# Yawning/secp256k1-voi

Hardware: AMD Instinct MI355X
Metric: secp256k1 ECDSA verifications/sec at batch=2^20 per GPU (higher is better)
Workload: dtype u32; 1 GPU; 2^20 ECDSA verifies (u1*G+u2*P per lane) per GPU (BASELINE config 2), 65536 distinct keys per GPU, all valid, low-s; parallelism=shard1, inputs=resident in HBM, collective=one all-gather per step: bitmap shard + valid count of every rank, gt_bits=26, gt_bits_at_first_call=20, gt_bytes=43822088192, numa_node=1, cpus_bound=128

## Files before the change

### include/secp256k1_voi_amd.h

```cpp
#ifndef SECP256K1_VOI_AMD_H
#define SECP256K1_VOI_AMD_H

#include <stddef.h>
#include <stdint.h>

#ifdef __cplusplus
extern "C" {
#endif

typedef struct s2k_ctx s2k_ctx;

enum {
  S2K_OK = 0,
  S2K_ERR_NO_DEVICE = -1,
  S2K_ERR_HIP = -2,
  S2K_ERR_ARG = -3,
  S2K_ERR_NOMEM = -4,
  S2K_PENDING = 1
};

#define S2K_ECDSA_REJECT_MALLEABLE 1u
#define S2K_ECDSA_FORCE_COMPLETE 0x80000000u
#define S2K_ECDSA_FORCE_WORKLIST 0x40000000u

// ... 330 lines not shown
int s2k_ct_scalar_set_bytes(const uint8_t src32[32], uint8_t out32[32], uint64_t *did_reduce);
int s2k_ct_fe_op(int op, const uint8_t a32[32], const uint8_t b32[32], uint8_t out32[32], uint64_t *flag);
uint64_t s2k_ct_debug_fe_mul_count(void);

enum {
  S2K_OP_MUL = 0,
  S2K_OP_SQR = 1,
  S2K_OP_ADD = 2,
  S2K_OP_SUB = 3,
  S2K_OP_NEG = 4,
  S2K_OP_INV = 5,
  S2K_OP_SQRT = 6
};
int s2k_fp_op_batch(s2k_ctx *ctx, int op, size_t n, const uint8_t *a, const uint8_t *b, uint8_t *out, uint8_t *flag);
int s2k_fn_op_batch(s2k_ctx *ctx, int op, size_t n, const uint8_t *a, const uint8_t *b, uint8_t *out, uint8_t *flag);
int s2k_fn_split_glv_batch(s2k_ctx *ctx, size_t n, const uint8_t *k, uint8_t *k1, uint8_t *k2);

enum {
  S2K_HP_MUL = 0, S2K_HP_SQR, S2K_HP_MUL_PLUS, S2K_HP_SQR_PLUS, S2K_HP_MUL_ADD_MUL, S2K_HP_MUL_ADD_SQR,
  S2K_HP_ADD, S2K_HP_NEGATE, S2K_HP_HALF, S2K_HP_NORMALIZE, S2K_HP_COND_NEGATE1, S2K_HP_INV, S2K_HP_SQRT,
  S2K_HP_EQ, S2K_HP_MUL_SMALL21, S2K_HP_NORMALIZE_WEAK, S2K_HP_JDBL, S2K_HP_JADD, S2K_HP_PT29_DBL,
  S2K_HP_PT29_ADD, S2K_HP_PT29_ADD_MIXED,
  S2K_HP_INV_GCD,
  S2K_HP_JADD_FULL,
  S2K_HP_PT29Q_DBL, S2K_HP_PT29Q_ADD,
  S2K_HP_XYZZ_ADD,
  S2K_HP_XYZZ_ROUND,
  S2K_HP_FER_MUL, S2K_HP_FER_MUL_PLUS, S2K_HP_FER_MUL_ADD_MUL, S2K_HP_FER_SMALL, S2K_HP_PT29R_DBL, S2K_HP_PT29R_ADD, S2K_HP_FER_SWAPS,
  S2K_HP_SC26_MUL, S2K_HP_SC26_SQR, S2K_HP_SC26_TO_MONT, S2K_HP_SC26_TO_SC, S2K_HP_SC26_INV, S2K_HP_SC26_CHAIN,
  S2K_HP_SC_MONTMUL, S2K_HP_SC_TO_MONT, S2K_HP_SC_MONT_INV, S2K_HP_SC_ADD, S2K_HP_SC_NEG, S2K_HP_SC_REDUCE_ONCE,
  S2K_HP_SC_GT_HALF_N,
  S2K_HP_AFF_DBL, S2K_HP_AFF_ADD,
  S2K_HP_XYZZ_ADD_FIRST,
  S2K_HP_PT29R_ADD_B3
};
int s2k_fp_op_batch_ex(s2k_ctx *ctx, uint32_t impl, int op, uint32_t lazy, size_t n, const uint8_t *const in[5],
                       uint8_t *out, uint8_t *out2, uint8_t *flag);
int s2k_fn_split_glv_batch_ex(s2k_ctx *ctx, uint32_t impl, size_t n, const uint8_t *k, uint8_t *k1, uint8_t *k2,
                              uint8_t *signs);

int s2k_generator_window_bits(void);
int s2k_debug_gtable_entry(s2k_ctx *ctx, unsigned i, unsigned d, uint8_t *out64);

#ifdef __cplusplus
}
#endif
#endif
```

### secp256k1_voi_amd/__init__.py

```python
from __future__ import annotations

import ctypes as C
import os
import subprocess

import numpy as np

if "GPU_MAX_HW_QUEUES" not in os.environ:
    os.environ["GPU_MAX_HW_QUEUES"] = "8"
    import sys as _sys
    _t = _sys.modules.get("torch")
    if _t is not None and getattr(_t, "cuda", None) is not None and _t.cuda.is_initialized():
        import warnings
        warnings.warn("secp256k1_voi_amd: the HIP runtime was initialised before this package was imported, so "
                      "GPU_MAX_HW_QUEUES=8 comes too late; streams of the engine may share hardware queues "
                      "(export GPU_MAX_HW_QUEUES=8 in the environment instead)", RuntimeWarning)

_HERE = os.path.dirname(os.path.abspath(__file__))
LIB_PATH = os.environ.get("S2K_LIB") or os.path.join(_HERE, "libsecp256k1_voi_amd.so")
CSRC = os.path.join(_HERE, "csrc")

REJECT_MALLEABLE = 1
BIP0066 = 2
FORCE_COMPLETE = 0x80000000
FORCE_WORKLIST = 0x40000000
ENCODING_ASN1, ENCODING_COMPACT, ENCODING_COMPACT_RECOVERABLE = 0, 1, 2

OP_MUL, OP_SQR, OP_ADD, OP_SUB, OP_NEG, OP_INV, OP_SQRT = range(7)
IMPL_COMPLETE, IMPL_FAST = 0, 1
CTX_WAIT_TABLES = 1
KEYS_OFF, KEYS_AUTO, KEYS_ALWAYS, KEYS_ADAPTIVE = 0, 1, 2, 3
LADDER_COMB, LADDER_WINDOW = 0, 1
KEYSET_AUTO, KEYSET_CHUNKS, KEYSET_JOINT, KEYSET_JOINT5, KEYSET_JOINT6, KEYSET_COMB = 0, 1, 2, 3, 4, 5
(HP_MUL, HP_SQR, HP_MUL_PLUS, HP_SQR_PLUS, HP_MUL_ADD_MUL, HP_MUL_ADD_SQR, HP_ADD, HP_NEGATE, HP_HALF, HP_NORMALIZE,
 HP_COND_NEGATE1, HP_INV, HP_SQRT, HP_EQ, HP_MUL_SMALL21, HP_NORMALIZE_WEAK, HP_JDBL, HP_JADD, HP_PT29_DBL, HP_PT29_ADD,
 HP_PT29_ADD_MIXED, HP_INV_GCD, HP_JADD_FULL, HP_PT29Q_DBL, HP_PT29Q_ADD, HP_XYZZ_ADD, HP_XYZZ_ROUND,
 HP_FER_MUL, HP_FER_MUL_PLUS, HP_FER_MUL_ADD_MUL, HP_FER_SMALL, HP_PT29R_DBL, HP_PT29R_ADD, HP_FER_SWAPS,
 HP_SC26_MUL, HP_SC26_SQR, HP_SC26_TO_MONT, HP_SC26_TO_SC, HP_SC26_INV, HP_SC26_CHAIN,
 HP_SC_MONTMUL, HP_SC_TO_MONT, HP_SC_MONT_INV, HP_SC_ADD, HP_SC_NEG, HP_SC_REDUCE_ONCE, HP_SC_GT_HALF_N,
 HP_AFF_DBL, HP_AFF_ADD, HP_XYZZ_ADD_FIRST, HP_PT29R_ADD_B3) = range(51)
KEYSET_LADDER_LANE, KEYSET_LADDER_ROW = 0, 1
H2C_SSWU_RO, H2C_SSWU_NU = 0, 1

IDENTITY = bytes(65)


def pinned_array(shape, dtype=np.uint8) -> np.ndarray:
    import weakref
    lib = load_library()
    nbytes = int(np.prod(shape)) * np.dtype(dtype).itemsize
    p = lib.s2k_host_alloc(max(nbytes, 1))
    if not p:
        raise EngineError("s2k_host_alloc failed")
    buf = (C.c_uint8 * max(nbytes, 1)).from_address(p)
    weakref.finalize(buf, lib.s2k_host_free, p)
    return np.frombuffer(buf, dtype=dtype, count=int(np.prod(shape))).reshape(shape)


def page_aligned_array(shape, dtype=np.uint8) -> np.ndarray:
    import mmap
    nbytes = int(np.prod(shape)) * np.dtype(dtype).itemsize
    page = mmap.PAGESIZE
    m = mmap.mmap(-1, max((nbytes + page - 1) // page * page, page))
    return np.frombuffer(m, dtype=dtype, count=int(np.prod(shape))).reshape(shape)


def host_register(a: np.ndarray) -> None:
    import mmap
    lib = load_library()
    nbytes, base = a.nbytes, a
    while getattr(base, "base", None) is not None:
        base = base.base
    if isinstance(base, memoryview):
# ... 191 lines not shown
    lib.s2k_group_keyset_create.argtypes = [vp, sz, vp, ci, vp]
    lib.s2k_group_keyset_destroy.argtypes = [vp]
    lib.s2k_group_keyset_destroy.restype = None
    lib.s2k_group_keyset_size.argtypes = [vp]
    lib.s2k_group_keyset_size.restype = sz
    lib.s2k_group_keyset_layout.argtypes = [vp]
    lib.s2k_group_keyset_device_bytes.argtypes = [vp]
    lib.s2k_group_keyset_device_bytes.restype = sz
    lib.s2k_group_ecdsa_verify_batch_keyset.argtypes = [vp, vp, sz, vp, vp, vp, vp, u32, vp]
    lib.s2k_group_ecdsa_verify_batch_keyset_submit.argtypes = [vp, vp, sz, vp, vp, vp, vp, u32, vp, vp]
    lib.s2k_group_ecdsa_verify_batch.argtypes = [vp, sz, vp, vp, vp, vp, u32, vp]
    lib.s2k_group_ecdsa_verify_batch_submit.argtypes = [vp, sz, vp, vp, vp, vp, u32, vp, C.POINTER(u64)]
    lib.s2k_group_wait.argtypes = [vp, u64]
    lib.s2k_group_ecdsa_verify_encoded_batch.argtypes = [vp, sz, vp, vp, vp, vp, vp, vp, ci, sz, u32, vp]
    lib.s2k_group_ecdsa_verify_encoded_batch_submit.argtypes = [vp, sz, vp, vp, vp, vp, vp, vp, ci, sz, u32, vp, C.POINTER(u64)]
    lib.s2k_group_member_stats.argtypes = [vp, vp]
    lib.s2k_schnorr_verify_batch.argtypes = [vp, sz, vp, vp, vp, sz, vp, u32, vp]
    lib.s2k_schnorr_verify_batch_device.argtypes = [vp, sz, vp, vp, vp, sz, vp, u32, vp, vp]
    lib.s2k_schnorr_verify_batch_keyset.argtypes = [vp, vp, sz, vp, vp, vp, sz, vp, u32, vp]
    lib.s2k_schnorr_verify_batch_keyset_device.argtypes = [vp, vp, sz, vp, vp, vp, sz, vp, u32, vp, vp]
    lib.s2k_schnorr_verify_batch_keyset_submit.argtypes = [vp, vp, sz, vp, vp, vp, sz, vp, u32, vp, vp]
    lib.s2k_schnorr_verify_batch_keyset_bykey.argtypes = [vp, vp, sz, vp, vp, vp, sz, vp, u32, vp]
    lib.s2k_schnorr_verify_batch_keyset_bykey_device.argtypes = [vp, vp, sz, vp, vp, vp, sz, vp, u32, vp, vp]
    lib.s2k_schnorr_verify_batch_keyset_bykey_submit.argtypes = [vp, vp, sz, vp, vp, vp, sz, vp, u32, vp, vp]
    lib.s2k_schnorr_batch_verify_rlc.argtypes = [vp, sz, vp, vp, vp, sz, vp, vp, C.POINTER(ci)]
    lib.s2k_schnorr_batch_verify_rlc_device.argtypes = [vp, sz, vp, vp, vp, sz, vp, vp, C.POINTER(ci), vp]
    lib.s2k_schnorr_verify_batch_bisect.argtypes = [vp, sz, vp, vp, vp, sz, vp, vp, vp, vp]
    lib.s2k_schnorr_verify_batch_bisect_device.argtypes = [vp, sz, vp, vp, vp, sz, vp, vp, vp, vp, vp]
    lib.s2k_scalar_base_mult_batch.argtypes = [vp, sz, vp, vp]
    lib.s2k_scalar_mult_batch.argtypes = [vp, sz, vp, vp, vp]
    lib.s2k_double_scalar_mult_basepoint_batch.argtypes = [vp, sz, vp, vp, vp, vp]
    lib.s2k_double_scalar_mult_basepoint_batch_ex.argtypes = [vp, u32, sz, vp, vp, vp, vp]
    lib.s2k_fp_op_batch_ex.argtypes = [vp, u32, ci, u32, sz, vp, vp, vp, vp]
    lib.s2k_fn_split_glv_batch_ex.argtypes = [vp, u32, sz, vp, vp, vp, vp]
    lib.s2k_point_add_batch.argtypes = [vp, sz, vp, vp, vp]
    lib.s2k_point_double_batch.argtypes = [vp, sz, vp, vp]
    lib.s2k_point_decode_batch.argtypes = [vp, sz, sz, vp, vp, vp]
    lib.s2k_multi_scalar_mult.argtypes = [vp, sz, vp, vp, vp]
    lib.s2k_multi_scalar_mult_device.argtypes = [vp, sz, vp, vp, vp, vp]
    lib.s2k_multi_scalar_mult_segments.argtypes = [vp, sz, vp, vp, sz, vp, vp]
    lib.s2k_multi_scalar_mult_segments_device.argtypes = [vp, sz, vp, vp, sz, vp, vp, vp]
    lib.s2k_debug_msm_segments_plan.argtypes = [sz, sz, vp, u32, C.c_uint64, vp, sz, vp, vp, vp, vp]
    lib.s2k_pointset_create.argtypes = [vp, sz, vp, ci, C.POINTER(vp)]
    lib.s2k_pointset_destroy.argtypes = [vp]
    lib.s2k_pointset_destroy.restype = None
    lib.s2k_pointset_size.argtypes = [vp]
    lib.s2k_pointset_size.restype = sz
    lib.s2k_pointset_window_bits.argtypes = [vp]
    lib.s2k_pointset_device_bytes.argtypes = [vp]
    lib.s2k_pointset_device_bytes.restype = sz
    lib.s2k_pointset_geometry.argtypes = [ci, vp]
    lib.s2k_keyset_geometry.argtypes = [ci, vp]
    lib.s2k_debug_pointset_entry.argtypes = [vp, sz, C.c_uint, C.c_uint, vp]
    lib.s2k_debug_pointset_check_args.argtypes = [sz, sz, ci, sz, vp]
    lib.s2k_pointset_multi_scalar_mult_segments.argtypes = [vp, vp, sz, vp, vp, sz, vp, vp]
    lib.s2k_pointset_multi_scalar_mult_segments_device.argtypes = [vp, vp, sz, vp, vp, sz, vp, vp, vp]
    lib.s2k_h2c_dst_prime.argtypes = [C.c_char_p, sz, C.c_char_p, C.POINTER(sz)]
    lib.s2k_expand_message_xmd_batch.argtypes = [vp, sz, C.c_char_p, sz, vp, vp, sz, sz, vp]
    lib.s2k_map_to_curve_batch.argtypes = [vp, sz, sz, sz, vp, vp]
    lib.s2k_hash_to_curve_batch.argtypes = [vp, ci, sz, C.c_char_p, sz, vp, vp, sz, vp]
    lib.s2k_hash_to_curve_batch_device.argtypes = [vp, ci, sz, C.c_char_p, sz, vp, vp, sz, sz, vp, vp]
    lib.s2k_fp_op_batch.argtypes = [vp, ci, sz, vp, vp, vp, vp]
    lib.s2k_fn_op_batch.argtypes = [vp, ci, sz, vp, vp, vp, vp]
    lib.s2k_fn_split_glv_batch.argtypes = [vp, sz, vp, vp, vp]
    lib.s2k_debug_gtable_entry.argtypes = [vp, C.c_uint, C.c_uint, vp]
    lib.s2k_ct_scalar_mult.argtypes = [C.c_char_p, C.c_char_p, C.c_char_p]
# ... 58 lines not shown
    "s2k_ctx_set_key_grouping", "s2k_ctx_set_keyed_ladder", "s2k_ctx_last_keyed_ladder", "s2k_ctx_key_grouping_stats", "s2k_ctx_key_grouping_adaptive",
    "s2k_ecdsa_verify_batch", "s2k_ecdsa_verify_batch_device", "s2k_ecdsa_workspace_bytes", "s2k_ctx_device_bytes",
    "s2k_keyset_create", "s2k_keyset_create_ex", "s2k_keyset_layout", "s2k_keyset_geometry", "s2k_keyset_destroy", "s2k_keyset_size", "s2k_keyset_device_bytes", "s2k_keyset_valid_keys",
    "s2k_ecdsa_verify_batch_keyset", "s2k_ecdsa_verify_batch_keyset_device", "s2k_ecdsa_verify_batch_keyset_submit",
    "s2k_keyset_index_geometry", "s2k_keyset_index_create", "s2k_keyset_index_info", "s2k_keyset_lookup", "s2k_keyset_lookup_device",
    "s2k_ecdsa_verify_batch_keyset_bykey", "s2k_ecdsa_verify_batch_keyset_bykey_device", "s2k_ecdsa_verify_batch_keyset_bykey_submit",
    "s2k_schnorr_verify_batch_keyset_bykey", "s2k_schnorr_verify_batch_keyset_bykey_device", "s2k_schnorr_verify_batch_keyset_bykey_submit",
    "s2k_pack_valid_device", "s2k_host_alloc", "s2k_host_free", "s2k_host_register", "s2k_host_unregister", "s2k_ecdsa_recover_batch", "s2k_ecdsa_recover_batch_device",
    "s2k_ecdsa_batch_verify_rlc", "s2k_ecdsa_batch_verify_rlc_device",
    "s2k_ecdsa_verify_recoverable_batch_bisect", "s2k_ecdsa_verify_recoverable_batch_bisect_device",
    "s2k_parse_asn1_signature", "s2k_parse_compact_signature", "s2k_is_valid_signature_encoding_bip0066",
    "s2k_ecdsa_verify_encoded_batch",
    "s2k_ecdsa_verify_encoded_batch_keyset", "s2k_ecdsa_verify_encoded_batch_keyset_submit", "s2k_ctx_last_encoded_keyset_stats",
    "s2k_ecdsa_verify_batch_submit", "s2k_ecdsa_verify_encoded_batch_submit", "s2k_wait", "s2k_poll", "s2k_wait_all",
    "s2k_device_count", "s2k_group_create", "s2k_group_destroy", "s2k_group_size", "s2k_group_last_error",
    "s2k_group_set_key_grouping", "s2k_group_set_small_batch_max", "s2k_group_set_mid_batch_max", "s2k_group_ecdsa_verify_batch", "s2k_group_ecdsa_verify_batch_submit", "s2k_group_wait",
    "s2k_group_ecdsa_verify_encoded_batch", "s2k_group_ecdsa_verify_encoded_batch_submit",
    "s2k_group_member_stats", "s2k_group_schnorr_batch_verify_rlc", "s2k_group_multi_scalar_mult",
    "s2k_group_keyset_create", "s2k_group_keyset_destroy", "s2k_group_keyset_size", "s2k_group_keyset_layout", "s2k_group_keyset_device_bytes",
    "s2k_group_ecdsa_verify_batch_keyset", "s2k_group_ecdsa_verify_batch_keyset_submit",
    "s2k_schnorr_verify_batch", "s2k_schnorr_verify_batch_device",
    "s2k_schnorr_verify_batch_keyset", "s2k_schnorr_verify_batch_keyset_device", "s2k_schnorr_verify_batch_keyset_submit",
    "s2k_schnorr_batch_verify_rlc", "s2k_schnorr_batch_verify_rlc_device",
    "s2k_schnorr_verify_batch_bisect", "s2k_schnorr_verify_batch_bisect_device",
    "s2k_scalar_base_mult_batch", "s2k_scalar_mult_batch", "s2k_double_scalar_mult_basepoint_batch",
    "s2k_point_add_batch", "s2k_point_double_batch", "s2k_point_decode_batch",
    "s2k_multi_scalar_mult", "s2k_multi_scalar_mult_device",
    "s2k_multi_scalar_mult_segments", "s2k_multi_scalar_mult_segments_device", "s2k_debug_msm_segments_plan",
    "s2k_pointset_create", "s2k_pointset_destroy", "s2k_pointset_size", "s2k_pointset_window_bits", "s2k_pointset_device_bytes",
    "s2k_pointset_geometry", "s2k_debug_pointset_entry", "s2k_debug_pointset_check_args",
    "s2k_pointset_multi_scalar_mult_segments", "s2k_pointset_multi_scalar_mult_segments_device",
    "s2k_h2c_dst_prime", "s2k_expand_message_xmd_batch", "s2k_map_to_curve_batch", "s2k_hash_to_curve_batch", "s2k_hash_to_curve_batch_device",
    "s2k_fp_op_batch", "s2k_fn_op_batch", "s2k_fn_split_glv_batch", "s2k_debug_gtable_entry", "s2k_generator_window_bits",
    "s2k_double_scalar_mult_basepoint_batch_ex", "s2k_fp_op_batch_ex", "s2k_fn_split_glv_batch_ex",
    "s2k_ct_scalar_mult", "s2k_ct_scalar_base_mult", "s2k_ct_ecdh", "s2k_ct_ecdsa_sign_raw", "s2k_ct_debug_fe_mul_count",
    "s2k_ct_multi_scalar_mult",
    "s2k_device_pci_bus_id", "s2k_device_numa_node", "s2k_bind_thread_to_node", "s2k_topology_prefer_node", "s2k_topology_node_count",
    "s2k_topology_numa_node_of_pci", "s2k_topology_node_cpus", "s2k_ctx_ticket_timing", "s2k_ticket_times",
    "s2k_group_member_stats_ex", "s2k_group_gt_wait", "s2k_group_shard_size", "s2k_group_host_alloc", "s2k_group_host_free",
    "s2k_ctx_set_small_batch_max", "s2k_ctx_set_mid_batch_max", "s2k_ctx_create_ex", "s2k_set_generator_table_budget", "s2k_set_table_memory_budgets", "s2k_ctx_gt_info", "s2k_ctx_gt_note", "s2k_ctx_gt_wait",
    "s2k_group_create_ex", "s2k_debug_gt_swap_in_call",
    "s2k_ctx_set_keyset_small_batch_max", "s2k_ctx_last_keyset_ladder", "s2k_group_set_keyset_small_batch_max",
    "s2k_ct_point_add", "s2k_ct_point_double", "s2k_ct_point_subtract", "s2k_ct_point_negate", "s2k_ct_point_conditional_negate",
    "s2k_ct_point_conditional_select", "s2k_ct_point_equal", "s2k_ct_point_is_identity", "s2k_ct_point_is_y_odd",
    "s2k_ct_scalar_op", "s2k_ct_scalar_conditional_select", "s2k_ct_scalar_conditional_negate", "s2k_ct_scalar_predicate",
    "s2k_ct_scalar_set_bytes", "s2k_ct_fe_op",
]


def _arr(x, width, n=None):
    if isinstance(x, (list, tuple)):
        x = b"".join(x)
    if isinstance(x, (bytes, bytearray, memoryview)):
        a = np.frombuffer(bytes(x), dtype=np.uint8)
    else:
        a = np.ascontiguousarray(x, dtype=np.uint8).reshape(-1)
    if a.size % width:
        raise ValueError(f"buffer length {a.size} is not a multiple of {width}")
    a = a.reshape(-1, width)
    if n is not None and a.shape[0] != n:
        raise ValueError(f"length mismatch: expected {n} items, got {a.shape[0]}")
    return np.ascontiguousarray(a)


def parse_asn1_signature(der: bytes):
    r, s = C.create_string_buffer(32), C.create_string_buffer(32)
    return (r.raw, s.raw) if load_library().s2k_parse_asn1_signature(der, len(der), r, s) == 0 else None
# ... 796 lines not shown
        out = self._points_out(n)
        self._check(self._lib.s2k_scalar_mult_batch(self._h, n, k.ctypes.data, points.ctypes.data, out.ctypes.data))
        return out

    def double_scalar_mult_basepoint_batch(self, u1, u2, points):
        u1 = _arr(u1, 32)
        n = u1.shape[0]
        u2, points = _arr(u2, 32, n), _arr(points, 65, n)
        out = self._points_out(n)
        self._check(self._lib.s2k_double_scalar_mult_basepoint_batch(self._h, n, u1.ctypes.data, u2.ctypes.data,
                                                                     points.ctypes.data, out.ctypes.data))
        return out

    def double_scalar_mult_basepoint_batch_ex(self, impl, u1, u2, points):
        u2 = _arr(u2, 32)
        n = u2.shape[0]
        points = _arr(points, 65, n)
        u1a = _arr(u1, 32, n) if u1 is not None else None
        out = self._points_out(n)
        self._check(self._lib.s2k_double_scalar_mult_basepoint_batch_ex(self._h, impl, n,
                                                                        u1a.ctypes.data if u1a is not None else None,
                                                                        u2.ctypes.data, points.ctypes.data, out.ctypes.data))
        return out

    def fp_op_batch_ex(self, op, operands, lazy=0):
        ops = [(_arr(x, 32) if x is not None else None) for x in operands] + [None] * (5 - len(operands))
        n = ops[0].shape[0]
        ptrs = (C.c_void_p * 5)(*[(x.ctypes.data if x is not None else None) for x in ops])
        out, out2, flag = (np.zeros((n, 32), dtype=np.uint8), np.zeros((n, 32), dtype=np.uint8), np.zeros(n, dtype=np.uint8))
        self._check(self._lib.s2k_fp_op_batch_ex(self._h, IMPL_FAST, op, lazy, n, ptrs, out.ctypes.data, out2.ctypes.data,
                                                 flag.ctypes.data))
        return out, out2, flag

    def fn_split_glv_odd_batch(self, k):
        k = _arr(k, 32)
        n = k.shape[0]
        k1, k2, sg = np.zeros((n, 32), np.uint8), np.zeros((n, 32), np.uint8), np.zeros(n, np.uint8)
        self._check(self._lib.s2k_fn_split_glv_batch_ex(self._h, IMPL_FAST, n, k.ctypes.data, k1.ctypes.data, k2.ctypes.data,
                                                        sg.ctypes.data))
        return k1, k2, sg

    def point_add_batch(self, a, b):
        a = _arr(a, 65)
        n = a.shape[0]
        b = _arr(b, 65, n)
        out = self._points_out(n)
        self._check(self._lib.s2k_point_add_batch(self._h, n, a.ctypes.data, b.ctypes.data, out.ctypes.data))
        return out

    def point_double_batch(self, a):
        a = _arr(a, 65)
        out = self._points_out(a.shape[0])
        self._check(self._lib.s2k_point_double_batch(self._h, a.shape[0], a.ctypes.data, out.ctypes.data))
        return out

    def multi_scalar_mult(self, scalars, points) -> bytes:
        scalars = _arr(scalars, 32)
        n = scalars.shape[0]
        points = _arr(points, 65, n)
        out = np.zeros(65, dtype=np.uint8)
        self._check(self._lib.s2k_multi_scalar_mult(self._h, n, scalars.ctypes.data if n else None,
                                                    points.ctypes.data if n else None, out.ctypes.data))
        return out.tobytes()

    def multi_scalar_mult_device(self, n, d_scalars, d_points, d_out65, stream=0):
        self._check(self._lib.s2k_multi_scalar_mult_device(self._h, int(n), d_scalars, d_points, d_out65, stream))
# ... 417 lines not shown
```

### secp256k1_voi_amd/csrc/engine.hip

```cpp
#include <hip/hip_runtime.h>

#include <cstdarg>
#include <cstdio>
#include <cstdlib>
#include <cstring>
#include <new>

#include <sys/random.h>
#include <unistd.h>

#include <atomic>
#include <chrono>
#include <condition_variable>
#include <mutex>
#include <thread>

#include "engine_internal.h"
#include "keyset_index.h"
#include "fe.h"
#include "fe29_inv.h"
#include "jacobian29.h"
#include "xyzz29.h"
#include "lane_tables.h"
#include "pt29.h"
// ... 619 lines not shown
    const uint4* kt = kg.ktab + (size_t)kg.ptab[idx] * (G::SLOTS * 8);
    {
      fe29 lx, ly;
      ke_load_xy(kt + (size_t)(neg1 == neg2 ? G::LEAD : G::LEAD + 1) * 8, false, lx, ly);
      acc.x = lx;
      acc.y = fe29_cond_negate1(ly, neg1);
      acc.z = fe29_one();
    }
    __shared__ uint32_t cols[G::SPACING][256];
    {
      uint32_t t1[G::TEETH], t2[G::TEETH];
#pragma unroll
      for (int t = 0; t < G::TEETH; ++t) {
        const int bit = G::SPACING * t + 1, limb = bit >> 5, sh = bit & 31;
        uint32_t v1 = k1.v[limb] >> sh, v2 = k2.v[limb] >> sh;
        if (sh > 32 - G::SPACING) {
          v1 |= k1.v[limb + 1] << (32 - sh);
          v2 |= k2.v[limb + 1] << (32 - sh);
        }
        t1[t] = v1 & ((1u << G::SPACING) - 1u);
        t2[t] = v2 & ((1u << G::SPACING) - 1u);
      }
#pragma unroll
      for (int j = 0; j < G::SPACING; ++j) {
        uint32_t w = 0;
#pragma unroll
        for (int t = 0; t < G::TEETH; ++t) w |= (((t1[t] >> j) & 1u) << t) | (((t2[t] >> j) & 1u) << (8 + t));
        cols[j][threadIdx.x] = w;
      }
    }
#pragma unroll 1
    for (int j = G::SPACING - 1;; --j) {
      const uint32_t w12 = cols[j][threadIdx.x], w1 = w12 & 127u, w2 = w12 >> 8;
#pragma unroll 1
      for (int t = 0; t < 2; ++t) {
        const uint32_t w = t ? w2 : w1;
        const bool top = (w & 64u) != 0;
        const bool neg = (t ? neg2 : neg1) != !top;
        const uint32_t entry = (top ? w : ~w) & 63u;
        fe29 x, y;
        ke_load_xy(kt + (size_t)entry * 8, t != 0, x, y);
        acc = jpt29_add_affine(acc, x, fe29_cond_negate1(y, neg));
      }
      if (j == 0) break;
      acc = jpt29_double(acc);
    }
    acc.z = fe29_mul(acc.z, ke_load(kt + (size_t)G::WENT * 8, G::W));
  } else if constexpr (KEYED) {
    using G = kt_geom<KEYSET ? KS_CHUNKS : KT_CHUNKS>;
    const uint4* kt = kg.ktab + (size_t)kg.ptab[idx] * (G::SLOTS * 8);
    const fe29 kw = ke_load(kt + (size_t)(G::SCR + G::W_SLOT / 3) * 8, G::W_SLOT % 3);
    xyzz29 xa;
    {
      fe29 lx, ly;
      if constexpr (JOINTW)
        jw_load(kg.jtab + (size_t)kg.ptab[idx] * kjw_geom<JW>::KEY_QUADS + (kjw_geom<JW>::LEAD + (neg1 == neg2 ? 0 : 1)) * kjw_geom<JW>::EQ, lx, ly);
      else
        ke_load_xy(kt + (size_t)(neg1 == neg2 ? G::LEAD : G::LEAD + 1) * 8, false, lx, ly);
      xa = xyzz29_from_affine(lx, fe29_cond_negate1(ly, neg1));
    }
    if constexpr (KEYSET) {
      uint32_t a[4], b[4];
#pragma unroll
      for (int w = 0; w < 4; ++w) {
        a[w] = (k1.v[w] >> 1) | (k1.v[w + 1] << 31);
        b[w] = (k2.v[w] >> 1) | (k2.v[w + 1] << 31);
      }
      [[maybe_unused]] const uint4* jt = JOINT ? kg.jtab + (size_t)kg.ptab[idx] * KJ_KEY_QUADS
                                        : JOINTW ? kg.jtab + (size_t)kg.ptab[idx] * kjw_geom<JW>::KEY_QUADS : nullptr;
      if constexpr (JOINTW) {
        using J = kjw_geom<JW>;
        constexpr uint32_t WM = (1u << JW) - 1u, NE = (uint32_t)J::NE;
        auto next_entry = [&](int c, bool& n1_out) -> uint32_t {
          const uint32_t w1 = a[0] & WM, w2 = b[0] & WM;
#pragma unroll
          for (int w = 0; w < 3; ++w) {
// ... 3684 lines not shown
```

### secp256k1_voi_amd/csrc/jacobian29.h

```cpp
#pragma once
#include "fe29.h"

namespace s2k {

struct jpt29 {
  fe29 x, y, z;
};

S2K_DEV jpt29 jpt29_double(const jpt29& p) {
  jpt29 r;
  r.z = fe29_mul(p.y, p.z);
  fe29 s = fe29_sqr(p.y);
  fe29 l = fe29_sqr(p.x);
  l = fe29_half(fe29_mul_int(l, 3));
  fe29 t = fe29_mul(fe29_negate(s, 1), p.x);
  r.x = fe29_sqr_plus(l, fe29_add(t, t));
  t = fe29_add(t, r.x);
  r.y = fe29_negate(fe29_mul_add_sqr(t, l, s), 1);
  return r;
}

S2K_DEV jpt29 jpt29_add_affine(const jpt29& p, const fe29& bx, const fe29& by, fe29* h_out = nullptr) {
  fe29 zz = fe29_sqr(p.z);
  fe29 nx = fe29_negate(p.x, 1);
  fe29 h = fe29_mul_plus(bx, zz, nx);
  fe29 ns = fe29_negate(fe29_mul(by, zz), 1);
  fe29 i = fe29_mul_plus(ns, p.z, p.y);
  jpt29 r;
  r.z = fe29_mul(p.z, h);
  fe29 h2 = fe29_sqr(h);
  fe29 h3 = fe29_mul(h2, fe29_negate(h, 1));
  fe29 t = fe29_mul(nx, h2);
  r.x = fe29_sqr_plus(i, fe29_add(fe29_add(h3, t), t));
  t = fe29_add(t, r.x);
  r.y = fe29_mul_add_mul(t, i, h3, p.y);
  if (h_out) *h_out = h;
  return r;
}

S2K_DEV jpt29 jpt29_add(const jpt29& p, const jpt29& q) {
  fe29 zz = fe29_sqr(q.z);
  fe29 zzz = fe29_mul(zz, q.z);
  jpt29 a;
  a.x = fe29_mul(p.x, zz);
  a.y = fe29_mul(p.y, zzz);
  a.z = p.z;
  jpt29 r = jpt29_add_affine(a, q.x, q.y);
  r.z = fe29_mul(r.z, q.z);
  return r;
}

}
```

### secp256k1_voi_amd/csrc/ops.hip

```cpp
#include <hip/hip_runtime.h>

#include <cstdint>
#include <cstring>

#include "aff29.h"
#include "complete_path.h"
#include "engine_internal.h"
#include "fe29_inv.h"
#include "jacobian29.h"
#include "pt29.h"
#include "pt29q.h"
#include "fe29r.h"
#include "xyzz29.h"
#include "sc26.h"

using namespace s2k;

extern "C" __attribute__((visibility("hidden"))) int s2k_internal_ensure_ws(s2k_ctx* ctx, size_t n);

S2K_DEV bool point_record_load(pt& p, const uint8_t* rec) {
  p = pt_identity();
  if (rec[0] == 0x00) return true;
  if (rec[0] != 0x04) return false;
  apt a;
// ... 351 lines not shown
  if (idx >= n) return;
  fe29 v[4];
#pragma unroll
  for (int j = 0; j < 4; ++j) {
    v[j] = fe29_zero();
    if (args.in[j]) {
      uint32_t w[8];
      load_be32(w, args.in[j] + idx * 32);
      v[j] = fe29_lazy_form(fe29_from_words(w), (lazy >> (4 * j)) & 15u);
    }
  }
  fe29 x = v[0], y = v[1];
#pragma unroll 1
  for (uint32_t i = 0; i < reps; ++i) {
    if (op == S2K_HP_AFF_DBL) {
      aff_double(x, y);
    } else {
      fe29 nx, ny;
      aff_add(x, y, v[2], v[3], nx, ny);
      x = nx;
      y = ny;
    }
  }
  uint32_t w[8];
  fe29_to_words(w, fe29_normalize(x));
  store_be32(out + idx * 32, w);
  if (out2) {
    fe29_to_words(w, fe29_normalize(y));
    store_be32(out2 + idx * 32, w);
  }
  if (flag) flag[idx] = 1;
}

__global__ void __launch_bounds__(256)
k_pt29q_op(int op, uint32_t lazy, uint32_t n, uint32_t reps, hp_args args, uint8_t* __restrict__ out, uint8_t* __restrict__ out2,
           uint8_t* __restrict__ flag) {
  const size_t t = (size_t)blockIdx.x * 256 + threadIdx.x;
  const size_t idx = t >> 2;
  const uint32_t q = (uint32_t)t & 3u;
  if (idx >= n) return;
  fe29 v[5];
#pragma unroll
  for (int j = 0; j < 5; ++j) {
    v[j] = fe29_zero();
    if (args.in[j]) {
      uint32_t w[8];
      load_be32(w, args.in[j] + idx * 32);
      v[j] = fe29_lazy_form(fe29_from_words(w), (lazy >> (4 * j)) & 15u);
    }
  }
  const fe29 &a = v[0], &b = v[1], &c = v[2], &d = v[3], &e = v[4];
  pt29 p, s;
  const bool p_inf = fe29_is_zero(c);
  const fe29 cn = fe29_normalize_weak(c);
  p.x = fe29_mul(a, cn);
  p.y = fe29_mul(b, cn);
  p.z = cn;
  s.x = fe29_mul(d, cn);
  s.y = fe29_mul(e, cn);
  s.z = cn;
  if (p_inf) {
    p = pt29_identity();
    s.x = fe29_normalize_weak(d);
    s.y = fe29_normalize_weak(e);
    s.z = fe29_one();
  }
// ... 392 lines not shown
  if (n > 0x7fffffffu) return fail(ctx, S2K_ERR_ARG, "batch too large");
  HIP_TRY(ctx, hipSetDevice(ctx->device));
  HIP_TRY(ctx, hipDeviceSynchronize());
  dev_buf din[5], dout, dout2, dflag;
  hp_args args;
  for (int j = 0; j < 5; ++j) {
    args.in[j] = nullptr;
    if (in[j]) {
      HIP_TRY(ctx, din[j].upload(in[j], n * 32));
      args.in[j] = (const uint8_t*)din[j].p;
    }
  }
  HIP_TRY(ctx, dout.alloc(n * 32));
  if (out2) HIP_TRY(ctx, dout2.alloc(n * 32));
  if (flag) HIP_TRY(ctx, dflag.alloc(n));
  if ((op >= S2K_HP_FER_MUL && op <= S2K_HP_FER_SWAPS) || op == S2K_HP_PT29R_ADD_B3)
    k_pt29r_op<<<blocks_for(64 * n), 256>>>(op, lazy, (uint32_t)n, reps ? reps : 1u, args, (uint8_t*)dout.p, (uint8_t*)dout2.p, (uint8_t*)dflag.p);
  else if (op == S2K_HP_AFF_DBL || op == S2K_HP_AFF_ADD)
    k_aff_op<<<blocks_for(n), 256>>>(op, lazy, (uint32_t)n, reps ? reps : 1u, args, (uint8_t*)dout.p, (uint8_t*)dout2.p, (uint8_t*)dflag.p);
  else if (op >= S2K_HP_SC26_MUL && op <= S2K_HP_SC_GT_HALF_N)
    k_sc_op<<<blocks_for(n), 256>>>(op, lazy, (uint32_t)n, reps ? reps : 1u, args, (uint8_t*)dout.p, (uint8_t*)dout2.p, (uint8_t*)dflag.p);
  else if (op == S2K_HP_PT29Q_DBL || op == S2K_HP_PT29Q_ADD)
    k_pt29q_op<<<blocks_for(4 * n), 256>>>(op, lazy, (uint32_t)n, reps ? reps : 1u, args, (uint8_t*)dout.p, (uint8_t*)dout2.p, (uint8_t*)dflag.p);
  else
    k_fp29_op<<<blocks_for(n), 256>>>(op, lazy, (uint32_t)n, args, (uint8_t*)dout.p, (uint8_t*)dout2.p, (uint8_t*)dflag.p);
  HIP_TRY(ctx, hipGetLastError());
  HIP_TRY(ctx, hipDeviceSynchronize());
  HIP_TRY(ctx, hipMemcpy(out, dout.p, n * 32, hipMemcpyDeviceToHost));
  if (out2) HIP_TRY(ctx, hipMemcpy(out2, dout2.p, n * 32, hipMemcpyDeviceToHost));
  if (flag) HIP_TRY(ctx, hipMemcpy(flag, dflag.p, n, hipMemcpyDeviceToHost));
  return S2K_OK;
}

int s2k_fn_split_glv_batch_ex(s2k_ctx* ctx, uint32_t impl, size_t n, const uint8_t* k, uint8_t* k1, uint8_t* k2, uint8_t* signs) {
  if (!ctx) return fail(nullptr, S2K_ERR_ARG, "ctx is NULL");
  if (impl != S2K_IMPL_FAST) return fail(ctx, S2K_ERR_ARG, "s2k_fn_split_glv_batch_ex serves S2K_IMPL_FAST only");
  if (n == 0) return S2K_OK;
  if (!k || !k1 || !k2 || !signs) return fail(ctx, S2K_ERR_ARG, "null buffer");
  HIP_TRY(ctx, hipSetDevice(ctx->device));
  HIP_TRY(ctx, hipDeviceSynchronize());
  dev_buf dk, d1, d2, ds;
  HIP_TRY(ctx, dk.upload(k, n * 32));
  HIP_TRY(ctx, d1.alloc(n * 32));
  HIP_TRY(ctx, d2.alloc(n * 32));
  HIP_TRY(ctx, ds.alloc(n));
  k_split_glv_odd<<<blocks_for(n), 256>>>((uint32_t)n, (const uint8_t*)dk.p, (uint8_t*)d1.p, (uint8_t*)d2.p, (uint8_t*)ds.p);
  HIP_TRY(ctx, hipGetLastError());
  HIP_TRY(ctx, hipDeviceSynchronize());
  HIP_TRY(ctx, hipMemcpy(k1, d1.p, n * 32, hipMemcpyDeviceToHost));
  HIP_TRY(ctx, hipMemcpy(k2, d2.p, n * 32, hipMemcpyDeviceToHost));
  HIP_TRY(ctx, hipMemcpy(signs, ds.p, n, hipMemcpyDeviceToHost));
  return S2K_OK;
}

int s2k_pack_valid_device(s2k_ctx* ctx, size_t n, const void* d_valid, void* d_bitmap, void* d_count,
                          void* hip_stream) {
  if (!ctx) return fail(nullptr, S2K_ERR_ARG, "ctx is NULL");
  if (!d_count) return fail(ctx, S2K_ERR_ARG, "null count buffer");
  hipStream_t st = (hipStream_t)hip_stream;
  HIP_TRY(ctx, hipSetDevice(ctx->device));
  HIP_TRY(ctx, hipMemsetAsync(d_count, 0, 8, st));
  if (n == 0) return S2K_OK;
  if (!d_valid || !d_bitmap) return fail(ctx, S2K_ERR_ARG, "null buffer");
  k_pack_valid<<<blocks_for((n + 8 * PACK_BYTES - 1) / (8 * PACK_BYTES)), 256, 0, st>>>((uint32_t)n, (const uint8_t*)d_valid, (uint8_t*)d_bitmap,
                                                        (unsigned long long*)d_count);
  HIP_TRY(ctx, hipGetLastError());
// ... 21 lines not shown
```

Baseline: 286.2 million verifications/s.

## Add two table points as a co-Z pair before adding to accumulator

In the keyset ladder loop, the two affine table entries per column are first summed together with a co-Z style pair addition. The accumulator is then rescaled by the pair's H^2/H^3, receives one mixed addition, and has its Z multiplied by H. This replaces two mixed Jacobian additions per column, aiming to cut field multiplications in the inner loop. A test kernel and API entry (JADD_PAIR) are added to check the new formula. The pair formula does not handle equal or opposite table points, which could be a correctness edge case.

```diff
diff --git a/include/secp256k1_voi_amd.h b/include/secp256k1_voi_amd.h
--- a/include/secp256k1_voi_amd.h
+++ b/include/secp256k1_voi_amd.h
@@ -386,10 +386,13 @@
   S2K_HP_SC_GT_HALF_N,
   S2K_HP_AFF_DBL, S2K_HP_AFF_ADD,
   S2K_HP_XYZZ_ADD_FIRST,
-  S2K_HP_PT29R_ADD_B3
+  S2K_HP_PT29R_ADD_B3,
+  S2K_HP_JADD_PAIR
 };
 int s2k_fp_op_batch_ex(s2k_ctx *ctx, uint32_t impl, int op, uint32_t lazy, size_t n, const uint8_t *const in[5],
                        uint8_t *out, uint8_t *out2, uint8_t *flag);
+int s2k_fp_op_batch_ex8(s2k_ctx *ctx, uint32_t impl, int op, uint32_t lazy, uint32_t reps, size_t n,
+                        const uint8_t *const in[8], uint8_t *out, uint8_t *out2, uint8_t *flag);
 int s2k_fn_split_glv_batch_ex(s2k_ctx *ctx, uint32_t impl, size_t n, const uint8_t *k, uint8_t *k1, uint8_t *k2,
                               uint8_t *signs);
 
diff --git a/secp256k1_voi_amd/__init__.py b/secp256k1_voi_amd/__init__.py
--- a/secp256k1_voi_amd/__init__.py
+++ b/secp256k1_voi_amd/__init__.py
@@ -38,7 +38,7 @@
  HP_FER_MUL, HP_FER_MUL_PLUS, HP_FER_MUL_ADD_MUL, HP_FER_SMALL, HP_PT29R_DBL, HP_PT29R_ADD, HP_FER_SWAPS,
  HP_SC26_MUL, HP_SC26_SQR, HP_SC26_TO_MONT, HP_SC26_TO_SC, HP_SC26_INV, HP_SC26_CHAIN,
  HP_SC_MONTMUL, HP_SC_TO_MONT, HP_SC_MONT_INV, HP_SC_ADD, HP_SC_NEG, HP_SC_REDUCE_ONCE, HP_SC_GT_HALF_N,
- HP_AFF_DBL, HP_AFF_ADD, HP_XYZZ_ADD_FIRST, HP_PT29R_ADD_B3) = range(51)
+ HP_AFF_DBL, HP_AFF_ADD, HP_XYZZ_ADD_FIRST, HP_PT29R_ADD_B3, HP_JADD_PAIR) = range(52)
 KEYSET_LADDER_LANE, KEYSET_LADDER_ROW = 0, 1
 H2C_SSWU_RO, H2C_SSWU_NU = 0, 1
 
@@ -296,6 +296,7 @@
     lib.s2k_double_scalar_mult_basepoint_batch.argtypes = [vp, sz, vp, vp, vp, vp]
     lib.s2k_double_scalar_mult_basepoint_batch_ex.argtypes = [vp, u32, sz, vp, vp, vp, vp]
     lib.s2k_fp_op_batch_ex.argtypes = [vp, u32, ci, u32, sz, vp, vp, vp, vp]
+    lib.s2k_fp_op_batch_ex8.argtypes = [vp, u32, ci, u32, u32, sz, vp, vp, vp, vp]
     lib.s2k_fn_split_glv_batch_ex.argtypes = [vp, u32, sz, vp, vp, vp, vp]
     lib.s2k_point_add_batch.argtypes = [vp, sz, vp, vp, vp]
     lib.s2k_point_double_batch.argtypes = [vp, sz, vp, vp]
@@ -420,7 +421,7 @@
     "s2k_pointset_multi_scalar_mult_segments", "s2k_pointset_multi_scalar_mult_segments_device",
     "s2k_h2c_dst_prime", "s2k_expand_message_xmd_batch", "s2k_map_to_curve_batch", "s2k_hash_to_curve_batch", "s2k_hash_to_curve_batch_device",
     "s2k_fp_op_batch", "s2k_fn_op_batch", "s2k_fn_split_glv_batch", "s2k_debug_gtable_entry", "s2k_generator_window_bits",
-    "s2k_double_scalar_mult_basepoint_batch_ex", "s2k_fp_op_batch_ex", "s2k_fn_split_glv_batch_ex",
+    "s2k_double_scalar_mult_basepoint_batch_ex", "s2k_fp_op_batch_ex", "s2k_fp_op_batch_ex8", "s2k_fn_split_glv_batch_ex",
     "s2k_ct_scalar_mult", "s2k_ct_scalar_base_mult", "s2k_ct_ecdh", "s2k_ct_ecdsa_sign_raw", "s2k_ct_debug_fe_mul_count",
     "s2k_ct_multi_scalar_mult",
     "s2k_device_pci_bus_id", "s2k_device_numa_node", "s2k_bind_thread_to_node", "s2k_topology_prefer_node", "s2k_topology_node_count",
@@ -1283,6 +1284,15 @@
                                                  flag.ctypes.data))
         return out, out2, flag
 
+    def fp_op_batch_ex8(self, op, operands, lazy=0, reps=0):
+        ops = [(_arr(x, 32) if x is not None else None) for x in operands] + [None] * (8 - len(operands))
+        n = ops[0].shape[0]
+        ptrs = (C.c_void_p * 8)(*[(x.ctypes.data if x is not None else None) for x in ops])
+        out, out2, flag = (np.zeros((n, 32), dtype=np.uint8), np.zeros((n, 32), dtype=np.uint8), np.zeros(n, dtype=np.uint8))
+        self._check(self._lib.s2k_fp_op_batch_ex8(self._h, IMPL_FAST, op, lazy, reps, n, ptrs, out.ctypes.data, out2.ctypes.data,
+                                                  flag.ctypes.data))
+        return out, out2, flag
+
     def fn_split_glv_odd_batch(self, k):
         k = _arr(k, 32)
         n = k.shape[0]
diff --git a/secp256k1_voi_amd/csrc/engine.hip b/secp256k1_voi_amd/csrc/engine.hip
--- a/secp256k1_voi_amd/csrc/engine.hip
+++ b/secp256k1_voi_amd/csrc/engine.hip
@@ -675,16 +675,15 @@
 #pragma unroll 1
     for (int j = G::SPACING - 1;; --j) {
       const uint32_t w12 = cols[j][threadIdx.x], w1 = w12 & 127u, w2 = w12 >> 8;
-#pragma unroll 1
-      for (int t = 0; t < 2; ++t) {
-        const uint32_t w = t ? w2 : w1;
-        const bool top = (w & 64u) != 0;
-        const bool neg = (t ? neg2 : neg1) != !top;
-        const uint32_t entry = (top ? w : ~w) & 63u;
-        fe29 x, y;
-        ke_load_xy(kt + (size_t)entry * 8, t != 0, x, y);
-        acc = jpt29_add_affine(acc, x, fe29_cond_negate1(y, neg));
-      }
+      const bool top1 = (w1 & 64u) != 0, top2 = (w2 & 64u) != 0;
+      const bool n1 = neg1 != !top1, n2 = neg2 != !top2;
+      fe29 x1, y1, x2, y2;
+      ke_load_xy(kt + (size_t)((top1 ? w1 : ~w1) & 63u) * 8, false, x1, y1);
+      ke_load_xy(kt + (size_t)((top2 ? w2 : ~w2) & 63u) * 8, true, x2, y2);
+      const coz29_sum t = coz29_pair_sum(x1, y1, x2, fe29_cond_negate1(y2, n1 != n2));
+      acc = jpt29_rescale(acc, t.hh, t.hhh);
+      acc = jpt29_add_affine(acc, t.x, fe29_cond_negate1(t.ny, !n1));
+      acc.z = fe29_mul(acc.z, t.h);
       if (j == 0) break;
       acc = jpt29_double(acc);
     }
diff --git a/secp256k1_voi_amd/csrc/jacobian29.h b/secp256k1_voi_amd/csrc/jacobian29.h
--- a/secp256k1_voi_amd/csrc/jacobian29.h
+++ b/secp256k1_voi_amd/csrc/jacobian29.h
@@ -50,4 +50,29 @@
   return r;
 }
 
+struct coz29_sum {
+  fe29 x, ny;
+  fe29 h, hh, hhh;
+};
+S2K_DEV coz29_sum coz29_pair_sum(const fe29& x1, const fe29& y1, const fe29& x2, const fe29& y2) {
+  coz29_sum t;
+  t.h = fe29_normalize_weak(fe29_add(x2, fe29_negate(x1, 1)));
+  t.hh = fe29_sqr(t.h);
+  const fe29 b = fe29_mul(x1, t.hh);
+  const fe29 c = fe29_mul(x2, t.hh);
+  const fe29 nb = fe29_negate(b, 1);
+  t.hhh = fe29_add(c, nb);
+  const fe29 dy = fe29_normalize_weak(fe29_add(y2, fe29_negate(y1, 1)));
+  t.x = fe29_sqr_plus(dy, fe29_negate(fe29_add(b, c), 2));
+  t.ny = fe29_mul_add_mul(dy, fe29_add(t.x, nb), y1, t.hhh);
+  return t;
 }
+S2K_DEV jpt29 jpt29_rescale(const jpt29& p, const fe29& zz, const fe29& zzz) {
+  jpt29 r;
+  r.x = fe29_mul(p.x, zz);
+  r.y = fe29_mul(p.y, zzz);
+  r.z = p.z;
+  return r;
+}
+
+}
diff --git a/secp256k1_voi_amd/csrc/ops.hip b/secp256k1_voi_amd/csrc/ops.hip
--- a/secp256k1_voi_amd/csrc/ops.hip
+++ b/secp256k1_voi_amd/csrc/ops.hip
@@ -407,6 +407,64 @@
   if (flag) flag[idx] = 1;
 }
 
+struct hp_args8 {
+  const uint8_t* in[8];
+};
+__global__ void __launch_bounds__(256)
+k_pair_op(uint32_t lazy, uint32_t n, uint32_t reps, hp_args8 args, uint8_t* __restrict__ out, uint8_t* __restrict__ out2,
+          uint8_t* __restrict__ flag) {
+  const size_t idx = (size_t)blockIdx.x * 256 + threadIdx.x;
+  if (idx >= n) return;
+  fe29 v[8];
+#pragma unroll
+  for (int j = 0; j < 8; ++j) {
+    v[j] = fe29_zero();
+    if (args.in[j]) {
+      uint32_t w[8];
+      load_be32(w, args.in[j] + idx * 32);
+      v[j] = fe29_lazy_form(fe29_from_words(w), (lazy >> (4 * j)) & 7u);
+    }
+  }
+  jpt29 acc;
+  if ((lazy >> 8) & 8u) {
+    acc.x = v[0];
+    acc.y = v[1];
+    acc.z = fe29_one();
+  } else {
+    const fe29 zz = fe29_sqr(v[2]);
+    acc.x = fe29_mul(v[0], zz);
+    acc.y = fe29_mul(v[1], fe29_mul(zz, v[2]));
+    acc.z = fe29_normalize_weak(v[2]);
+  }
+  const fe29 &x1 = v[3], &y1 = v[4], &x2 = v[5], &y2 = v[6];
+  const bool n1 = (v[7].n[0] & 1u) != 0, n2 = (v[7].n[0] & 2u) != 0;
+#pragma unroll 1
+  for (uint32_t i = 0; i < (reps ? reps : 1u); ++i) {
+    const coz29_sum t = coz29_pair_sum(x1, y1, x2, fe29_cond_negate1(y2, n1 != n2));
+    acc = jpt29_rescale(acc, t.hh, t.hhh);
+    acc = jpt29_add_affine(acc, t.x, fe29_cond_negate1(t.ny, !n1));
+    acc.z = fe29_mul(acc.z, t.h);
+    if (reps) acc = jpt29_double(acc);
+  }
+  fe29 r = fe29_zero(), r2 = fe29_zero();
+  uint8_t f = 1;
+  if (fe29_is_zero(acc.z)) {
+    f = 0;
+  } else {
+    const fe29 zi = fe29_inv(acc.z), zi2 = fe29_sqr(zi);
+    r = fe29_mul(acc.x, zi2);
+    r2 = fe29_mul(fe29_mul(acc.y, zi2), zi);
+  }
+  uint32_t w[8];
+  fe29_to_words(w, fe29_normalize(r));
+  store_be32(out + idx * 32, w);
+  if (out2) {
+    fe29_to_words(w, fe29_normalize(r2));
+    store_be32(out2 + idx * 32, w);
+  }
+  if (flag) flag[idx] = f;
+}
+
 __global__ void __launch_bounds__(256)
 k_pt29q_op(int op, uint32_t lazy, uint32_t n, uint32_t reps, hp_args args, uint8_t* __restrict__ out, uint8_t* __restrict__ out2,
            uint8_t* __restrict__ flag) {
@@ -865,6 +923,40 @@
   return S2K_OK;
 }
 
+int s2k_fp_op_batch_ex8(s2k_ctx* ctx, uint32_t impl, int op, uint32_t lazy, uint32_t reps, size_t n, const uint8_t* const in[8],
+                        uint8_t* out, uint8_t* out2, uint8_t* flag) {
+  if (!ctx) return fail(nullptr, S2K_ERR_ARG, "ctx is NULL");
+  if (impl != S2K_IMPL_FAST) return fail(ctx, S2K_ERR_ARG, "s2k_fp_op_batch_ex8 serves S2K_IMPL_FAST only");
+  if (op != S2K_HP_JADD_PAIR) return fail(ctx, S2K_ERR_ARG, "bad op");
+  if (n == 0) return S2K_OK;
+  if (!in || !out) return fail(ctx, S2K_ERR_ARG, "null buffer");
+  for (int j = 0; j < 8; ++j)
+    if (!in[j] && j != 2 && j != 7) return fail(ctx, S2K_ERR_ARG, "null buffer");
+  if (!in[2] && !((lazy >> 8) & 8u)) return fail(ctx, S2K_ERR_ARG, "no Z to lift P to");
+  if (n > 0x7fffffffu) return fail(ctx, S2K_ERR_ARG, "batch too large");
+  HIP_TRY(ctx, hipSetDevice(ctx->device));
+  HIP_TRY(ctx, hipDeviceSynchronize());
+  dev_buf din[8], dout, dout2, dflag;
+  hp_args8 args;
+  for (int j = 0; j < 8; ++j) {
+    args.in[j] = nullptr;
+    if (in[j]) {
+      HIP_TRY(ctx, din[j].upload(in[j], n * 32));
+      args.in[j] = (const uint8_t*)din[j].p;
+    }
+  }
+  HIP_TRY(ctx, dout.alloc(n * 32));
+  if (out2) HIP_TRY(ctx, dout2.alloc(n * 32));
+  if (flag) HIP_TRY(ctx, dflag.alloc(n));
+  k_pair_op<<<blocks_for(n), 256>>>(lazy, (uint32_t)n, reps, args, (uint8_t*)dout.p, (uint8_t*)dout2.p, (uint8_t*)dflag.p);
+  HIP_TRY(ctx, hipGetLastError());
+  HIP_TRY(ctx, hipDeviceSynchronize());
+  HIP_TRY(ctx, hipMemcpy(out, dout.p, n * 32, hipMemcpyDeviceToHost));
+  if (out2) HIP_TRY(ctx, hipMemcpy(out2, dout2.p, n * 32, hipMemcpyDeviceToHost));
+  if (flag) HIP_TRY(ctx, hipMemcpy(flag, dflag.p, n, hipMemcpyDeviceToHost));
+  return S2K_OK;
+}
+
 int s2k_fn_split_glv_batch_ex(s2k_ctx* ctx, uint32_t impl, size_t n, const uint8_t* k, uint8_t* k1, uint8_t* k2, uint8_t* signs) {
   if (!ctx) return fail(nullptr, S2K_ERR_ARG, "ctx is NULL");
   if (impl != S2K_IMPL_FAST) return fail(ctx, S2K_ERR_ARG, "s2k_fn_split_glv_batch_ex serves S2K_IMPL_FAST only");
```

New measurement: 302.6 million verifications/s, median of 6. 5.7% higher.
